# caishiqing/voice-tts

Measured on AMD Instinct MI355X. Metric: audio_seconds_per_second, higher is better.
Workload: dtype bf16

## Files before the change

### include/ixtts_hip.h

```cpp
#ifndef IXTTS_HIP_H
#define IXTTS_HIP_H

#include <stddef.h>
#include <stdint.h>

#ifdef __cplusplus
extern "C" {
#endif

#define IXTTS_OK 0
#define IXTTS_ERR_ARG (-1)
#define IXTTS_ERR_HIP (-2)
#define IXTTS_ERR_STATE (-3)
#define IXTTS_ERR_NOMEM (-4)
#define IXTTS_ERR_NAME (-5)

const char* ixtts_version(void);
const char* ixtts_last_error(void);

int ixtts_aa_snake_f32(const float* x_dev, float* y_dev, const float* up12_dev, const float* down12_dev,
                       const float* log_alpha_dev, const float* log_beta_dev, int B, int C, int T, void* stream);

size_t ixtts_attn_full_workspace_bytes(int B, int H, int T);
int ixtts_attn_full_f32(const float* q_dev, const float* k_dev, const float* v_dev, float* out_dev, int B, int H, int T,
// ... 114 lines not shown
int ixtts_gpt_beam_begin(ixtts_gpt* h, int num_beams, void* stream);
int ixtts_gpt_beam_decode(ixtts_gpt* h, int n_steps, const ixtts_sampler_cfg* sc, void* stream);
int ixtts_gpt_beam_read(ixtts_gpt* h, int max_new, int32_t* ids_host, int cap, int* n_ids, int* done, float* score,
                        float* beam_scores_host, int32_t* last_tokens_host, int32_t* beam_idx_host, void* stream);
int ixtts_gpt_beam_force(ixtts_gpt* h, const int32_t* picks_host, int n, void* stream);

int ixtts_gpt_beam_begin_group(ixtts_gpt* h, int group, int num_beams, uint64_t rng_stream, void* stream);
int ixtts_gpt_beam_park_group(ixtts_gpt* h, int group, void* stream);
int ixtts_gpt_beam_decode_groups(ixtts_gpt* h, int n_groups, int n_steps, const ixtts_sampler_cfg* sc, void* stream);
int ixtts_gpt_beam_read_group(ixtts_gpt* h, int group, int max_new, int32_t* ids_host, int cap, int* n_ids, int* done, float* score,
                              float* beam_scores_host, int32_t* last_tokens_host, int32_t* beam_idx_host, void* stream);
int ixtts_gpt_beam_force_group(ixtts_gpt* h, int group, const int32_t* picks_host, int n, void* stream);

int ixtts_gpt_latent(ixtts_gpt* h, const float* prefix_dev, int n_prefix, const int32_t* codes_dev, int n,
                     float* latent_dev, void* stream);

int ixtts_gpt_bench_gemv(ixtts_gpt* h, int which, int layer, int batch, void* stream);
double ixtts_gpt_step_bytes(const ixtts_gpt* h, int B, int S);

int ixtts_gpt_max_batch(void);

int ixtts_gpt_destroy(ixtts_gpt* h);

#define IXTTS_QWEN_TOPK_MAX 64
#define IXTTS_QWEN_MAX_EOS 8

typedef struct ixtts_qwen_cfg {
  int hidden_size;
  int layers;
  int heads;
// ... 42 lines not shown
```

### voice-tts_amd/_lib.py

```python
import ctypes as C
import os

HERE = os.path.dirname(os.path.abspath(__file__))
LIB_PATH = os.environ.get("IXTTS_LIB") or os.path.join(HERE, "libixtts_hip.so")

MAX_STAGES = 8
MAX_RESK = 4


class BigVGANCfg(C.Structure):
    _fields_ = [
        ("num_mels", C.c_int), ("upsample_initial_channel", C.c_int), ("n_stages", C.c_int),
        ("upsample_rates", C.c_int * MAX_STAGES), ("upsample_kernel_sizes", C.c_int * MAX_STAGES),
        ("n_resblock_kernels", C.c_int), ("resblock_kernel_sizes", C.c_int * MAX_RESK),
        ("resblock_dilations", (C.c_int * 3) * MAX_RESK), ("max_frames", C.c_int), ("fast_sin", C.c_int),
    ]


class GptCfg(C.Structure):
    _fields_ = [
        ("model_dim", C.c_int), ("layers", C.c_int), ("heads", C.c_int), ("n_mel_codes", C.c_int),
        ("n_mel_pos", C.c_int), ("n_text_tokens", C.c_int), ("n_text_pos", C.c_int),
        ("start_mel_token", C.c_int), ("stop_mel_token", C.c_int), ("max_seq", C.c_int),
        ("max_batch", C.c_int), ("weight_dtype", C.c_int),
# ... 75 lines not shown
    "ixtts_gpt_decode": (C.c_int, [_P, C.c_int, C.c_int, C.POINTER(SamplerCfg), _P]),
    "ixtts_gpt_read": (C.c_int, [_P, C.c_int, _P, C.c_int, C.POINTER(C.c_int), C.POINTER(C.c_int), _P]),
    "ixtts_gpt_read_logits": (C.c_int, [_P, C.c_int, _P, _P]),
    "ixtts_gpt_beam_begin": (C.c_int, [_P, C.c_int, _P]),
    "ixtts_gpt_beam_decode": (C.c_int, [_P, C.c_int, C.POINTER(SamplerCfg), _P]),
    "ixtts_gpt_beam_read": (C.c_int, [_P, C.c_int, _P, C.c_int, C.POINTER(C.c_int), C.POINTER(C.c_int), C.POINTER(C.c_float), _P, _P, _P, _P]),
    "ixtts_gpt_beam_force": (C.c_int, [_P, _P, C.c_int, _P]),
    "ixtts_gpt_beam_begin_group": (C.c_int, [_P, C.c_int, C.c_int, C.c_uint64, _P]),
    "ixtts_gpt_beam_park_group": (C.c_int, [_P, C.c_int, _P]),
    "ixtts_gpt_beam_decode_groups": (C.c_int, [_P, C.c_int, C.c_int, C.POINTER(SamplerCfg), _P]),
    "ixtts_gpt_beam_read_group": (C.c_int, [_P, C.c_int, C.c_int, _P, C.c_int, C.POINTER(C.c_int), C.POINTER(C.c_int), C.POINTER(C.c_float), _P, _P, _P, _P]),
    "ixtts_gpt_beam_force_group": (C.c_int, [_P, C.c_int, _P, C.c_int, _P]),
    "ixtts_gpt_read_probs": (C.c_int, [_P, C.c_int, _P, _P]),
    "ixtts_gpt_force_next": (C.c_int, [_P, C.c_int, C.c_int32, _P]),
    "ixtts_gpt_latent": (C.c_int, [_P, _P, C.c_int, _P, C.c_int, _P, _P]),
    "ixtts_gpt_bench_gemv": (C.c_int, [_P, C.c_int, C.c_int, C.c_int, _P]),
    "ixtts_gpt_step_bytes": (C.c_double, [_P, C.c_int, C.c_int]),
    "ixtts_gpt_max_batch": (C.c_int, []),
    "ixtts_gpt_destroy": (C.c_int, [_P]),
    "ixtts_qwen_create": (C.c_int, [C.POINTER(_P), C.POINTER(QwenCfg)]),
    "ixtts_qwen_set_tensor": (C.c_int, [_P, C.c_char_p, _P, C.POINTER(C.c_int64), C.c_int]),
    "ixtts_qwen_finalize": (C.c_int, [_P]),
    "ixtts_qwen_prefill": (C.c_int, [_P, _P, C.c_int, _P]),
    "ixtts_qwen_step": (C.c_int, [_P, C.c_int, C.POINTER(QwenSampling), _P]),
    "ixtts_qwen_read": (C.c_int, [_P, _P, C.c_int, C.POINTER(C.c_int), C.POINTER(C.c_int), _P]),
    "ixtts_qwen_generate": (C.c_int, [_P, C.c_int, C.POINTER(QwenSampling), _P, C.c_int, C.POINTER(C.c_int), C.POINTER(C.c_int), _P]),
    "ixtts_qwen_read_logits": (C.c_int, [_P, _P, _P]),
    "ixtts_qwen_read_kept": (C.c_int, [_P, _P, _P, C.c_int, C.POINTER(C.c_int), _P]),
    "ixtts_qwen_draw": (C.c_int, [_P, C.c_uint64, C.c_int, _P, _P]),
    "ixtts_qwen_step_bytes": (C.c_double, [_P, C.c_int]),
# ... 44 lines not shown
```

### voice-tts_amd/csrc/gpt_engine.h

```cpp
#pragma once
#include <map>
#include <string>
#include <vector>

#include "common.h"

namespace ixtts {

constexpr int MAXB = 16;
constexpr int MAXB_REG = 4;
constexpr int STEPS_PER_GRAPH = 8;
constexpr int BEAM_MAX = 4;
constexpr int MAXG = MAXB / 2;
constexpr int BEAM_LCP_STRIDE = BEAM_MAX * BEAM_MAX + BEAM_MAX;
constexpr int BEAM_FORCED_STRIDE = 2 * BEAM_MAX;

enum TKind { T_VEC = 0, T_MAT_T = 1, T_MAT_N = 2, T_EMB = 3 };

struct TDesc {
  size_t off = 0;
  int kind = T_VEC;
  int64_t d0 = 0, d1 = 0;
  size_t stage_off = 0;
  bool set = false;
// ... 48 lines not shown
  float* probs = nullptr;
  ixtts_sampler_cfg samp_host;
  float* scratch = nullptr;
  size_t scratch_floats = 0;
  hipStream_t cap_stream = nullptr;
  hipGraphExec_t step_exec[ixtts::MAXB + 1][ixtts::NBKT + 1] = {};
  hipGraphExec_t multi_exec[ixtts::MAXB + 1][ixtts::NBKT + 1] = {};
  bool mlp_fused = false;
  void* wprx = nullptr;
  float* mlp_part = nullptr;
  unsigned* mlp_ctr = nullptr;
  float* h2 = nullptr;
  float* hc = nullptr;
  bool wide = false;
  int pf_per = 2;
  bool attn_split = true;
  int attn_bucket = ixtts::NBKT;
  int host_prompt_len[ixtts::MAXB + 2];
  int host_gen_est[ixtts::MAXB + 2];
  int num_beams = 0;
  int beam_groups = 1;
  bool group_live[ixtts::MAXG] = {};
  bool group_begun[ixtts::MAXG] = {};
  unsigned long long* beam_stream = nullptr;
  float *beam_scores = nullptr, *hyp_score = nullptr, *hyp_worst = nullptr;
  int *beam_src = nullptr, *hyp_len = nullptr, *n_hyp = nullptr, *beam_done = nullptr, *beam_forced_flag = nullptr;
  int32_t *hyp_tok = nullptr, *beam_forced = nullptr;
  float* beam_cand_v = nullptr;
  int *beam_cand_i = nullptr, *beam_cand_n = nullptr;
  bool beam_every_row = false;
// ... 22 lines not shown
```

### voice-tts_amd/csrc/gpt_engine.hip

```cpp
#define IXTTS_ENGINE_TU 1
#include <type_traits>

#include "gpt_engine.h"
#include "gpt_kernels.h"
#include "gpt_wide.h"

using namespace ixtts;

#ifdef IXTTS_TRACE
static int g_trace_seq = 0;
#define IXTTS_TRACE_ARG , g_trace_seq++
#else
#define IXTTS_TRACE_ARG
#endif
template <typename WT, typename KVT, int K, int ROWS, int UNITS, int B, int INP, int EPI, int WPB = 4, bool XLDS = false>
static int launch_gemv(const GemvArgs& a, hipStream_t st) {
  auto kern = gemv_reg_kernel<WT, K, ROWS, UNITS, B, INP, EPI, KVT, WPB, XLDS>;
  const int n_units = (a.N + ROWS - 1) / ROWS;
  const int grid = ceil_div(n_units, WPB * UNITS);
  hipLaunchKernelGGL(kern, dim3(grid), dim3(64 * WPB), 0, st, a.wt, a.xin, a.bias, a.out, a.N, a.slot0, a.out_stride, a.smax, a.kcache, a.vcache,
                     a.cur_len, a.heads, a.nsplit, a.ln_w, a.ln_b, a.aux, a.xout IXTTS_PF_ARGS(a) IXTTS_TRACE_ARG);
  return IXTTS_OK;
}

// ... 472 lines not shown
  {
    int ones[MAXG];
    for (int g = 0; g < MAXG; ++g) ones[g] = 1;
    hipMemcpy(h->beam_done, ones, sizeof(ones), hipMemcpyHostToDevice);
    hipMemset(h->beam_forced_flag, 0, MAXG * 4);
    hipMemset(h->beam_stream, 0, MAXG * 8);
    hipMemset(h->n_hyp, 0, MAXG * 4);
    hipMemset(h->beam_lcp, 0, (size_t)MAXG * BEAM_LCP_STRIDE * 4);
    hipMemset(h->beam_src, 0, MAXB * 4);
  }
  if (hipStreamCreateWithFlags(&h->cap_stream, hipStreamNonBlocking) != hipSuccess) return fail("stream");
  if (const char* e = getenv("IXTTS_ATTN")) h->attn_split = strcmp(e, "legacy") != 0;
  h->wide = c->max_batch > MAXB_REG;
  if (const char* e = getenv("IXTTS_WIDE")) h->wide = h->wide || (strcmp(e, "1") == 0 && c->weight_dtype != IXTTS_DTYPE_F32);
  if (const char* e = getenv("IXTTS_BEAM_REORDER")) h->beam_every_row = strcmp(e, "full") == 0;
  if (const char* e = getenv("IXTTS_PF_KIB")) h->pf_per = atoi(e);
  if (h->wide) h->attn_split = false;
  memset(h->host_prompt_len, 0, sizeof(h->host_prompt_len));
  memset(h->host_gen_est, 0, sizeof(h->host_gen_est));
  *out = h;
  return IXTTS_OK;
}

extern "C" int ixtts_gpt_set_tensor(ixtts_gpt* h, const char* name, const float* data, const int64_t* shape, int ndim) {
  IX_ARG(h && name && data && shape, "gpt_set_tensor: null argument");
  auto it = h->tens.find(name);
  if (it == h->tens.end()) {
    set_error("gpt_set_tensor: unknown tensor '%s'", name);
    return IXTTS_ERR_NAME;
  }
// ... 564 lines not shown
  IX_ARG(n + 2 <= h->cfg.n_mel_pos, "gpt_latent: %d codes exceed the mel position table", n);
  IX_ARG(n_prefix + n + 2 < h->smax, "gpt_latent: sequence of %d rows exceeds max_seq %d", n_prefix + n + 2, h->smax);
  if (n == 0) return IXTTS_OK;
  hipStream_t st = (hipStream_t)stream;
  const int D = h->D;
  const int slot = h->slots - 1;
  const int rows = n_prefix + n;
  IX_HIP(hipMemcpyAsync(h->rx, prefix, (size_t)n_prefix * D * 4, hipMemcpyDeviceToDevice, st));
  IX_TRY(embed_mel_rows(h, h->rx + (size_t)n_prefix * D, codes, n, st));
  IX_TRY(forward_rows(h, slot, rows, 0, 0, st));
  IX_TRY(final_norm_rows(h, h->rx + (size_t)n_prefix * D, latent, n, st));
  IX_HIP(hipGetLastError());
  return IXTTS_OK;
}

extern "C" int ixtts_gpt_bench_gemv(ixtts_gpt* h, int which, int layer, int batch, void* stream) {
  NEED_READY(h, "gpt_bench_gemv");
  IX_ARG(layer >= 0 && layer < h->L && batch >= 1 && batch <= h->cfg.max_batch, "gpt_bench_gemv: bad argument");
  return do_gemv_which(h, which, layer, batch, (hipStream_t)stream);
}

extern "C" int ixtts_gpt_max_batch(void) { return MAXB; }

extern "C" double ixtts_gpt_step_bytes(const ixtts_gpt* h, int B, int S) {
  if (!h) return 0.0;
  const double D = h->D, FF = h->FF, V = h->V, L = h->L, es = (double)h->esize;
  double mat = L * (3 * D * D + D * D + 2 * D * FF) + V * D;
  double vec = L * (2 * D + 3 * D + D + 2 * D + FF + D) + 4 * D + V;
  double kv_read = (double)B * 2 * L * S * D * es;
  double kv_write = (double)B * 2 * L * D * es;
// ... 50 lines not shown
```

### voice-tts_amd/csrc/gpt_rows.hip

```cpp
#include "gpt_engine.h"
#include "gpt_kernels.h"

namespace ixtts {

typedef float f32x16 __attribute__((ext_vector_type(16)));
typedef __bf16 bf16x8 __attribute__((ext_vector_type(8)));
typedef _Float16 f16x8 __attribute__((ext_vector_type(8)));

template <typename ET>
struct RowsEl;
template <>
struct RowsEl<bf16> {
  typedef bf16x8 vec8;
  __device__ static __forceinline__ f32x16 mfma(const vec8& a, const vec8& b, const f32x16& c) { return __builtin_amdgcn_mfma_f32_32x32x16_bf16(a, b, c, 0, 0, 0); }
};
template <>
struct RowsEl<f16> {
  typedef f16x8 vec8;
  __device__ static __forceinline__ f32x16 mfma(const vec8& a, const vec8& b, const f32x16& c) { return __builtin_amdgcn_mfma_f32_32x32x16_f16(a, b, c, 0, 0, 0); }
};

__device__ __forceinline__ unsigned int pack_bf16x2(float a, float b) {
  const unsigned short lo = __builtin_bit_cast(unsigned short, (__bf16)a);
  const unsigned short hi = __builtin_bit_cast(unsigned short, (__bf16)b);
// ... 223 lines not shown

struct GemmArgs16 {
  const unsigned short* A;
  const unsigned short* wt;
  const float* bias;
  void* out;
  void* kcache;
  void* vcache;
  int T, N, K, pos0, smax, D;
};

__device__ __forceinline__ void glds16(const void* gsrc, void* lds_wave_base) {
  __builtin_amdgcn_global_load_lds((const __attribute__((address_space(1))) void*)gsrc, (__attribute__((address_space(3))) void*)lds_wave_base, 16, 0, 0);
}

constexpr int G16_NBUF = 2;
constexpr int G16_TILE = 128 * 64 * 2;
constexpr int G16_SMEM = G16_NBUF * 2 * G16_TILE;

template <int EPI, typename KVT>
__global__ __launch_bounds__(256) void gemm_rows_bf16_kernel(GemmArgs16 g) {
  using EL = RowsEl<KVT>;
  typedef typename EL::vec8 vec8;
  constexpr int BM = 128, BN = 128, BK = 64, TILE = G16_TILE, NBUF = G16_NBUF;
  extern __shared__ __attribute__((aligned(1024))) unsigned char smem_raw[];
  unsigned char (*smem)[2][TILE] = reinterpret_cast<unsigned char (*)[2][TILE]>(smem_raw);
  const int tid = threadIdx.x, lane = tid & 63, wave = tid >> 6;
  const int wm = wave >> 1, wn = wave & 1;
  const int l31 = lane & 31, lh = lane >> 5;
  const int m0 = blockIdx.y * BM, n0 = blockIdx.x * BN;

  f32x16 acc[2][2];
#pragma unroll
  for (int mi = 0; mi < 2; ++mi)
#pragma unroll
    for (int j = 0; j < 2; ++j)
#pragma unroll
      for (int r = 0; r < 16; ++r) acc[mi][j][r] = 0.f;

  const unsigned short* asrc[4];
  const unsigned short* wsrc[4];
#pragma unroll
  for (int i = 0; i < 4; ++i) {
    const int row = (wave * 4 + i) * 8 + (lane >> 3);
    const int gran = (lane & 7) ^ ((row >> 1) & 7);
    asrc[i] = g.A + (size_t)min(m0 + row, g.T - 1) * g.K + gran * 8;
    wsrc[i] = g.wt + (size_t)min(n0 + row, g.N - 1) * g.K + gran * 8;
  }
  auto issue = [&](int kt, int buf) {
#pragma unroll
    for (int i = 0; i < 4; ++i) {
      glds16(asrc[i] + kt * BK, &smem[buf][0][(wave * 4 + i) * 1024]);
      glds16(wsrc[i] + kt * BK, &smem[buf][1][(wave * 4 + i) * 1024]);
    }
  };
  const int nkt = g.K / BK;
#pragma unroll
  for (int p = 0; p < NBUF - 1; ++p) issue(min(p, nkt - 1), p);
  for (int kt = 0; kt < nkt; ++kt) {
    issue(min(kt + NBUF - 1, nkt - 1), (kt + NBUF - 1) % NBUF);
    static_assert(NBUF == 2, "the immediate below is 8 * (NBUF - 1)");
    asm volatile("s_waitcnt vmcnt(8)" ::: "memory");
    __builtin_amdgcn_s_barrier();
    const unsigned char* At = smem[kt % NBUF][0];
    const unsigned char* Wt = smem[kt % NBUF][1];
#pragma unroll
    for (int kk = 0; kk < BK / 16; ++kk) {
      vec8 a[2], b[2];
#pragma unroll
      for (int mi = 0; mi < 2; ++mi) {
        const int row = wm * 64 + mi * 32 + l31;
        a[mi] = *reinterpret_cast<const vec8*>(At + row * 128 + (((kk * 2 + lh) ^ ((row >> 1) & 7)) << 4));
      }
#pragma unroll
      for (int j = 0; j < 2; ++j) {
        const int row = wn * 64 + j * 32 + l31;
        b[j] = *reinterpret_cast<const vec8*>(Wt + row * 128 + (((kk * 2 + lh) ^ ((row >> 1) & 7)) << 4));
      }
#pragma unroll
      for (int mi = 0; mi < 2; ++mi)
#pragma unroll
        for (int j = 0; j < 2; ++j) acc[mi][j] = EL::mfma(a[mi], b[j], acc[mi][j]);
    }
    __builtin_amdgcn_s_barrier();
  }
  float bias[2];
  int ncol[2];
#pragma unroll
  for (int j = 0; j < 2; ++j) {
    ncol[j] = n0 + wn * 64 + j * 32 + l31;
    bias[j] = g.bias[min(ncol[j], g.N - 1)];
  }
  if constexpr (EPI == RE_RESID) {
    float* xo = reinterpret_cast<float*>(g.out);
    float old[2][2][16];
#pragma unroll
    for (int mi = 0; mi < 2; ++mi)
#pragma unroll
      for (int j = 0; j < 2; ++j)
#pragma unroll
        for (int r = 0; r < 16; ++r) {
          const int m = min(m0 + wm * 64 + mi * 32 + (r & 3) + 8 * (r >> 2) + 4 * lh, g.T - 1);
          old[mi][j][r] = xo[(size_t)m * g.N + min(ncol[j], g.N - 1)];
        }
#pragma unroll
    for (int mi = 0; mi < 2; ++mi)
#pragma unroll
      for (int j = 0; j < 2; ++j)
#pragma unroll
        for (int r = 0; r < 16; ++r) {
          const int m = m0 + wm * 64 + mi * 32 + (r & 3) + 8 * (r >> 2) + 4 * lh;
          if (m < g.T && ncol[j] < g.N) xo[(size_t)m * g.N + ncol[j]] = old[mi][j][r] + (acc[mi][j][r] + bias[j]);
        }
  } else {
#pragma unroll
    for (int mi = 0; mi < 2; ++mi)
#pragma unroll
      for (int j = 0; j < 2; ++j) {
        const int n = ncol[j];
#pragma unroll
        for (int r = 0; r < 16; ++r) {
          const int m = m0 + wm * 64 + mi * 32 + (r & 3) + 8 * (r >> 2) + 4 * lh;
          if (m >= g.T || n >= g.N) continue;
          const float v = acc[mi][j][r] + bias[j];
          if constexpr (EPI == RE_GELU) {
            const float u2 = 1.5957691216057308f * (v + 0.044715f * v * v * v);
            store_kv(reinterpret_cast<KVT*>(g.out) + (size_t)m * g.N + n, v / (1.0f + __expf(-u2)));
          } else {
            if (n < g.D) {
              reinterpret_cast<float*>(g.out)[(size_t)m * g.D + n] = v;
            } else {
              const int which = n / g.D;
              const int c = n - which * g.D;
              const int hh = c / HD, d = c % HD;
              KVT* cache = reinterpret_cast<KVT*>(which == 1 ? g.kcache : g.vcache);
              store_kv(cache + ((size_t)hh * g.smax + g.pos0 + m) * HD + d, v);
            }
// ... 53 lines not shown
    const uint4 r = reinterpret_cast<const uint4*>(p)[i];
    v[8 * i] = lo_f16(r.x); v[8 * i + 1] = hi_f16(r.x); v[8 * i + 2] = lo_f16(r.y); v[8 * i + 3] = hi_f16(r.y);
    v[8 * i + 4] = lo_f16(r.z); v[8 * i + 5] = hi_f16(r.z); v[8 * i + 6] = lo_f16(r.w); v[8 * i + 7] = hi_f16(r.w);
  }
}
template <>
__device__ __forceinline__ void load_row16<bf16>(const bf16* p, float (&v)[16]) {
#pragma unroll
  for (int i = 0; i < 2; ++i) {
    const uint4 r = reinterpret_cast<const uint4*>(p)[i];
    v[8 * i] = lo_bf16(r.x); v[8 * i + 1] = hi_bf16(r.x); v[8 * i + 2] = lo_bf16(r.y); v[8 * i + 3] = hi_bf16(r.y);
    v[8 * i + 4] = lo_bf16(r.z); v[8 * i + 5] = hi_bf16(r.z); v[8 * i + 6] = lo_bf16(r.w); v[8 * i + 7] = hi_bf16(r.w);
  }
}

template <typename KVT, typename OT>
__global__ __launch_bounds__(256) void attn_rows_flash_kernel(AttnRowsArgs a) {
  __shared__ __attribute__((aligned(16))) float Ks[FR_KT * FR_KP];
  __shared__ __attribute__((aligned(16))) float Vs[FR_KT * HD];
  const int hh = blockIdx.x;
  const int lane = threadIdx.x & 63, wave = threadIdx.x >> 6;
  const int l31 = lane & 31, lh = lane >> 5;
  const int qw0 = blockIdx.y * 128 + wave * 32;
  const KVT* kb = reinterpret_cast<const KVT*>(a.kcache) + (size_t)hh * a.smax * HD;
  const KVT* vb = reinterpret_cast<const KVT*>(a.vcache) + (size_t)hh * a.smax * HD;
  const int last_key = a.pos0 + a.T - 1;

  float qr[HD / 2];
  {
    const int qi = min(qw0 + l31, a.T - 1);
    const float* qp = a.q + (size_t)qi * a.D + hh * HD + 4 * lh;
    const float qs = 0.125f * 1.4426950408889634f;
#pragma unroll
    for (int m = 0; m < HD / 8; ++m) {
      const float4 t = *reinterpret_cast<const float4*>(qp + 8 * m);
      qr[4 * m] = t.x * qs; qr[4 * m + 1] = t.y * qs; qr[4 * m + 2] = t.z * qs; qr[4 * m + 3] = t.w * qs;
    }
  }
  f32x16 ot[2];
#pragma unroll
  for (int j = 0; j < 2; ++j)
#pragma unroll
    for (int r = 0; r < 16; ++r) ot[j][r] = 0.f;
  float m_run = -INFINITY, l_run = 0.f;
  const int lim = a.pos0 + qw0 + l31;
  const int wave_lim = a.pos0 + min(qw0 + 31, a.T - 1);
  const int wg_lim = a.pos0 + min((int)blockIdx.y * 128 + 127, a.T - 1);
  const int t_first = (a.valid_from / FR_KT) * FR_KT;

  for (int t0 = t_first; t0 <= wg_lim; t0 += FR_KT) {
    __syncthreads();
    {
      const int key = threadIdx.x >> 2, c16 = (threadIdx.x & 3) * 16;
      const int t = min(max(t0 + key, a.valid_from), last_key);
      float kv[16], vv[16];
      load_row16<KVT>(kb + (size_t)t * HD + c16, kv);
      load_row16<KVT>(vb + (size_t)t * HD + c16, vv);
#pragma unroll
      for (int i = 0; i < 4; ++i) {
        *reinterpret_cast<float4*>(Ks + key * FR_KP + c16 + 4 * i) = make_float4(kv[4 * i], kv[4 * i + 1], kv[4 * i + 2], kv[4 * i + 3]);
        *reinterpret_cast<float4*>(Vs + key * HD + c16 + 4 * i) = make_float4(vv[4 * i], vv[4 * i + 1], vv[4 * i + 2], vv[4 * i + 3]);
      }
    }
    __syncthreads();
    if (t0 > wave_lim) continue;

    f32x16 st[2];
#pragma unroll
    for (int j = 0; j < 2; ++j)
#pragma unroll
      for (int r = 0; r < 16; ++r) st[j][r] = 0.f;
    const float* kp0 = Ks + l31 * FR_KP + 4 * lh;
    const float* kp1 = kp0 + 32 * FR_KP;
    float4 ka[2][2];
    ka[0][0] = *reinterpret_cast<const float4*>(kp0);
    ka[0][1] = *reinterpret_cast<const float4*>(kp1);
#pragma unroll
    for (int m = 0; m < HD / 8; ++m) {
      if (m + 1 < HD / 8) {
// ... 62 lines not shown
      ot[0] = __builtin_amdgcn_mfma_f32_32x32x2f32(va[s2 & 1][0], pv, ot[0], 0, 0, 0);
      ot[1] = __builtin_amdgcn_mfma_f32_32x32x2f32(va[s2 & 1][1], pv, ot[1], 0, 0, 0);
    }
  }
  const int qi = qw0 + l31;
  if (qi < a.T) {
    const float inv = l_run > 0.f ? 1.0f / l_run : 0.f;
    OT* op = reinterpret_cast<OT*>(a.out) + (size_t)qi * a.D + hh * HD;
#pragma unroll
    for (int j = 0; j < 2; ++j)
#pragma unroll
      for (int r = 0; r < 16; ++r) store_kv(op + j * 32 + (r & 3) + 8 * (r >> 2) + 4 * lh, ot[j][r] * inv);
  }
}

template <typename KVT, typename OT>
static void launch_attn_rows(ixtts_gpt* h, const AttnRowsArgs& a, hipStream_t st) {
  static const bool legacy = getenv("IXTTS_ROWS_ATTN") && !strcmp(getenv("IXTTS_ROWS_ATTN"), "legacy");
  if (legacy) hipLaunchKernelGGL((attn_rows_kernel<KVT, OT>), dim3(h->H, a.T), dim3(256), 0, st, a);
  else hipLaunchKernelGGL((attn_rows_flash_kernel<KVT, OT>), dim3(h->H, ceil_div(a.T, 128)), dim3(256), 0, st, a);
}

template <typename WT, typename KVT, int EPI>
static void launch_gemm(const GemmArgs& g, hipStream_t st) {
  if (g.T >= 512) {
    hipLaunchKernelGGL((gemm_rows_kernel<WT, EPI, KVT, 128>), dim3(ceil_div(g.N, GBN), ceil_div(g.T, 128)), dim3(256), 0, st, g);
  } else {
    hipLaunchKernelGGL((gemm_rows_kernel<WT, EPI, KVT, 64>), dim3(ceil_div(g.N, GBN), ceil_div(g.T, 64)), dim3(256), 0, st, g);
  }
}

template <typename WT, typename KVT, int D>
static int forward_rows_t(ixtts_gpt* h, int slot, int T, int pos0, int valid_from, hipStream_t st) {
  const size_t lstride = (size_t)h->slots * D * h->smax * sizeof(KVT);
  const size_t sstride = (size_t)D * h->smax * sizeof(KVT);
// ... 9 lines not shown
    AttnRowsArgs a;
    a.q = h->rq; a.kcache = kc; a.vcache = vc; a.out = h->ratt; a.T = T; a.D = D; a.smax = h->smax; a.pos0 = pos0; a.valid_from = valid_from;
    launch_attn_rows<KVT, float>(h, a, st);
    g.A = h->ratt; g.wt = A_PTR(o.wo); g.bias = A_F32(o.bo); g.out = h->rx; g.N = D; g.K = D;
    launch_gemm<WT, KVT, RE_RESID>(g, st);
    hipLaunchKernelGGL(ln_rows_kernel<D>, dim3(ceil_div(T, 4)), dim3(256), 0, st, h->rx, h->rxn, T);
    g.A = h->rxn; g.wt = A_PTR(o.wfc); g.bias = A_F32(o.bfc); g.out = h->rff; g.N = 4 * D; g.K = D;
    launch_gemm<WT, KVT, RE_GELU>(g, st);
    g.A = h->rff; g.wt = A_PTR(o.wpr); g.bias = A_F32(o.bpr); g.out = h->rx; g.N = D; g.K = 4 * D;
    launch_gemm<WT, KVT, RE_RESID>(g, st);
  }
  IX_HIP(hipGetLastError());
  return IXTTS_OK;
}

template <typename KVT, int D>
static int forward_rows_16(ixtts_gpt* h, int slot, int T, int pos0, int valid_from, hipStream_t st) {
  const size_t lstride = (size_t)h->slots * D * h->smax * sizeof(KVT);
  const size_t sstride = (size_t)D * h->smax * sizeof(KVT);
  KVT* xn16 = reinterpret_cast<KVT*>(h->rxn);
  KVT* att16 = reinterpret_cast<KVT*>(h->ratt);
  KVT* ff16 = reinterpret_cast<KVT*>(h->rff);
  const dim3 blk(256);
  auto grid = [&](int N) { return dim3(ceil_div(N, 128), ceil_div(T, 128)); };
  static bool attr_done = false;
  if (!attr_done) {
    IX_HIP(hipFuncSetAttribute((const void*)gemm_rows_bf16_kernel<RE_QKV, KVT>, hipFuncAttributeMaxDynamicSharedMemorySize, G16_SMEM));
    IX_HIP(hipFuncSetAttribute((const void*)gemm_rows_bf16_kernel<RE_RESID, KVT>, hipFuncAttributeMaxDynamicSharedMemorySize, G16_SMEM));
    IX_HIP(hipFuncSetAttribute((const void*)gemm_rows_bf16_kernel<RE_GELU, KVT>, hipFuncAttributeMaxDynamicSharedMemorySize, G16_SMEM));
    attr_done = true;
  }
  for (int l = 0; l < h->L; ++l) {
    const LayerOff& o = h->lo[l];
    uint8_t* kc = (uint8_t*)h->kc + l * lstride + slot * sstride;
    uint8_t* vc = (uint8_t*)h->vc + l * lstride + slot * sstride;
    hipLaunchKernelGGL((ln_rows_kernel<D, KVT>), dim3(ceil_div(T, 4)), blk, 0, st, h->rx, xn16, T);
    GemmArgs16 g;
    g.A = reinterpret_cast<const unsigned short*>(xn16); g.wt = reinterpret_cast<const unsigned short*>(A_PTR(o.wqkv)); g.bias = A_F32(o.bqkv);
    g.out = h->rq; g.kcache = kc; g.vcache = vc; g.T = T; g.N = 3 * D; g.K = D; g.pos0 = pos0; g.smax = h->smax; g.D = D;
    hipLaunchKernelGGL((gemm_rows_bf16_kernel<RE_QKV, KVT>), grid(g.N), blk, G16_SMEM, st, g);
    AttnRowsArgs a;
    a.q = h->rq; a.kcache = kc; a.vcache = vc; a.out = att16; a.T = T; a.D = D; a.smax = h->smax; a.pos0 = pos0; a.valid_from = valid_from;
    launch_attn_rows<KVT, KVT>(h, a, st);
    g.A = reinterpret_cast<const unsigned short*>(att16); g.wt = reinterpret_cast<const unsigned short*>(A_PTR(o.wo)); g.bias = A_F32(o.bo);
    g.out = h->rx; g.N = D; g.K = D;
    hipLaunchKernelGGL((gemm_rows_bf16_kernel<RE_RESID, KVT>), grid(g.N), blk, G16_SMEM, st, g);
    hipLaunchKernelGGL((ln_rows_kernel<D, KVT>), dim3(ceil_div(T, 4)), blk, 0, st, h->rx, xn16, T);
    g.A = reinterpret_cast<const unsigned short*>(xn16); g.wt = reinterpret_cast<const unsigned short*>(A_PTR(o.wfc)); g.bias = A_F32(o.bfc);
    g.out = ff16; g.N = 4 * D; g.K = D;
    hipLaunchKernelGGL((gemm_rows_bf16_kernel<RE_GELU, KVT>), grid(g.N), blk, G16_SMEM, st, g);
    g.A = reinterpret_cast<const unsigned short*>(ff16); g.wt = reinterpret_cast<const unsigned short*>(A_PTR(o.wpr)); g.bias = A_F32(o.bpr);
    g.out = h->rx; g.N = D; g.K = 4 * D;
    hipLaunchKernelGGL((gemm_rows_bf16_kernel<RE_RESID, KVT>), grid(g.N), blk, G16_SMEM, st, g);
  }
  IX_HIP(hipGetLastError());
  return IXTTS_OK;
}

int forward_rows(ixtts_gpt* h, int slot, int T, int pos0, int valid_from, hipStream_t st) {
  if (T <= 0) return IXTTS_OK;
  if (h->cfg.weight_dtype == IXTTS_DTYPE_F32) {
    return h->D == 1280 ? forward_rows_t<float, float, 1280>(h, slot, T, pos0, valid_from, st)
                        : forward_rows_t<float, float, 128>(h, slot, T, pos0, valid_from, st);
  }
  if (h->cfg.weight_dtype == IXTTS_DTYPE_F16)
    return h->D == 1280 ? forward_rows_16<f16, 1280>(h, slot, T, pos0, valid_from, st) : forward_rows_16<f16, 128>(h, slot, T, pos0, valid_from, st);
  return h->D == 1280 ? forward_rows_16<bf16, 1280>(h, slot, T, pos0, valid_from, st) : forward_rows_16<bf16, 128>(h, slot, T, pos0, valid_from, st);
}
// ... 31 lines not shown
```

### voice-tts_amd/gpt_engine.py

```python
import ctypes as C

import numpy as np
import torch

from . import _lib
from .weights import GPT_CFG

GPT_DTYPES = {"f32": 0, "bf16": 1, "f16": 2}


def _dtype_code(dtype):
    if dtype not in GPT_DTYPES:
        raise ValueError(f"GPT weight dtype {dtype!r}: expected one of " + ", ".join(GPT_DTYPES))
    return GPT_DTYPES[dtype]


def resolve_gpt_dtype(use_fp16, gpt_dtype=None, env=None):
    import os

    if gpt_dtype is None:
        gpt_dtype = (os.environ if env is None else env).get("IXTTS_GPT_DTYPE") or None
        if gpt_dtype is not None:
            gpt_dtype = gpt_dtype.strip().lower()
    if gpt_dtype is None:
# ... 136 lines not shown
        src = np.zeros(self._nb, np.int32)
        with torch.cuda.device(self.device):
            rc = _lib.lib().ixtts_gpt_beam_read_group(self._h, int(group), int(max_new), ids.ctypes.data, ids.size, C.byref(n), C.byref(done), C.byref(score),
                                                      bs.ctypes.data, lt.ctypes.data, src.ctypes.data, self._stream())
        _lib.check(rc, "ixtts_gpt_beam_read_group")
        return ids[: n.value].copy(), bool(done.value), float(score.value), bs, lt, src

    def latent(self, prefix, codes):
        p = prefix.to(self.device, torch.float32).contiguous()
        c = codes.to(self.device, torch.int32).contiguous()
        out = torch.empty(c.numel(), self.D, device=self.device, dtype=torch.float32)
        with torch.cuda.device(self.device):
            rc = _lib.lib().ixtts_gpt_latent(self._h, p.data_ptr(), p.shape[0], c.data_ptr(), c.numel(), out.data_ptr(), self._stream())
        _lib.check(rc, "ixtts_gpt_latent")
        self._keep2 = (p, c)
        return out

    def step_bytes(self, B, S):
        return _lib.lib().ixtts_gpt_step_bytes(self._h, B, S)

    def bench_gemv(self, which, layer, batch=1):
        with torch.cuda.device(self.device):
            _lib.check(_lib.lib().ixtts_gpt_bench_gemv(self._h, which, layer, batch, self._stream()), "ixtts_gpt_bench_gemv")

    def store_mel_emb(self, mel_emb):
        self.cached_mel_emb = mel_emb

    def generate(self, inputs, bos_token_id=None, pad_token_id=None, eos_token_id=None, attention_mask=None,
                 max_length=None, logits_processor=None, num_return_sequences=1, do_sample=True, top_p=1.0, top_k=0,
                 temperature=1.0, num_beams=1, repetition_penalty=1.0, length_penalty=0.0, sync_every=64,
# ... 86 lines not shown
```

Baseline: 41.31.

## Pick GEMM row tile shape by grid size and prefetch KV in flash attention

Parameterizes the prefill rows GEMM over tile shape and buffer count, adding 128x64 and 64x64 tiles with deeper pipelines and an M-fast grid. A heuristic picks the smaller tiles when the legacy 128x128 grid would launch too few workgroups to fill the GPU. The flash attention rows kernel now prefetches the next K/V tile into registers while computing the current one, and schedules row blocks in reverse order. A debug peek API and an IXTTS_ROWS=legacy fallback are also added. Smaller tiles reuse less data per load and add register pressure.

```diff
diff --git a/include/ixtts_hip.h b/include/ixtts_hip.h
--- a/include/ixtts_hip.h
+++ b/include/ixtts_hip.h
@@ -152,6 +152,8 @@
 
 int ixtts_gpt_latent(ixtts_gpt* h, const float* prefix_dev, int n_prefix, const int32_t* codes_dev, int n,
                      float* latent_dev, void* stream);
+
+int ixtts_gpt_peek(ixtts_gpt* h, int what, int layer, int slot, void* out_host, size_t bytes, void* stream);
 
 int ixtts_gpt_bench_gemv(ixtts_gpt* h, int which, int layer, int batch, void* stream);
 double ixtts_gpt_step_bytes(const ixtts_gpt* h, int B, int S);
diff --git a/voice-tts_amd/_lib.py b/voice-tts_amd/_lib.py
--- a/voice-tts_amd/_lib.py
+++ b/voice-tts_amd/_lib.py
@@ -113,6 +113,7 @@
     "ixtts_gpt_read_probs": (C.c_int, [_P, C.c_int, _P, _P]),
     "ixtts_gpt_force_next": (C.c_int, [_P, C.c_int, C.c_int32, _P]),
     "ixtts_gpt_latent": (C.c_int, [_P, _P, C.c_int, _P, C.c_int, _P, _P]),
+    "ixtts_gpt_peek": (C.c_int, [_P, C.c_int, C.c_int, C.c_int, _P, C.c_size_t, _P]),
     "ixtts_gpt_bench_gemv": (C.c_int, [_P, C.c_int, C.c_int, C.c_int, _P]),
     "ixtts_gpt_step_bytes": (C.c_double, [_P, C.c_int, C.c_int]),
     "ixtts_gpt_max_batch": (C.c_int, []),
diff --git a/voice-tts_amd/csrc/gpt_engine.h b/voice-tts_amd/csrc/gpt_engine.h
--- a/voice-tts_amd/csrc/gpt_engine.h
+++ b/voice-tts_amd/csrc/gpt_engine.h
@@ -86,6 +86,7 @@
   float* hc = nullptr;
   bool wide = false;
   int pf_per = 2;
+  bool rows_legacy = false;
   bool attn_split = true;
   int attn_bucket = ixtts::NBKT;
   int host_prompt_len[ixtts::MAXB + 2];
diff --git a/voice-tts_amd/csrc/gpt_engine.hip b/voice-tts_amd/csrc/gpt_engine.hip
--- a/voice-tts_amd/csrc/gpt_engine.hip
+++ b/voice-tts_amd/csrc/gpt_engine.hip
@@ -510,6 +510,7 @@
   h->wide = c->max_batch > MAXB_REG;
   if (const char* e = getenv("IXTTS_WIDE")) h->wide = h->wide || (strcmp(e, "1") == 0 && c->weight_dtype != IXTTS_DTYPE_F32);
   if (const char* e = getenv("IXTTS_BEAM_REORDER")) h->beam_every_row = strcmp(e, "full") == 0;
+  if (const char* e = getenv("IXTTS_ROWS")) h->rows_legacy = strcmp(e, "legacy") == 0;
   if (const char* e = getenv("IXTTS_PF_KIB")) h->pf_per = atoi(e);
   if (h->wide) h->attn_split = false;
   memset(h->host_prompt_len, 0, sizeof(h->host_prompt_len));
@@ -1104,6 +1105,25 @@
   return IXTTS_OK;
 }
 
+extern "C" int ixtts_gpt_peek(ixtts_gpt* h, int what, int layer, int slot, void* out_host, size_t bytes, void* stream) {
+  NEED_READY(h, "gpt_peek");
+  IX_ARG(out_host && what >= 0 && what <= 2, "gpt_peek: bad argument");
+  const uint8_t* src;
+  size_t cap;
+  if (what == 0) {
+    src = reinterpret_cast<const uint8_t*>(h->rx);
+    cap = (size_t)h->smax * h->D * 4;
+  } else {
+    IX_ARG(layer >= 0 && layer < h->L && slot >= 0 && slot < h->slots, "gpt_peek: layer %d / slot %d out of range", layer, slot);
+    cap = (size_t)h->D * h->smax * h->esize;
+    src = reinterpret_cast<const uint8_t*>(what == 1 ? h->kc : h->vc) + ((size_t)layer * h->slots + slot) * cap;
+  }
+  IX_ARG(bytes <= cap, "gpt_peek: %zu bytes asked of a region of %zu", bytes, cap);
+  IX_HIP(hipStreamSynchronize((hipStream_t)stream));
+  IX_HIP(hipMemcpy(out_host, src, bytes, hipMemcpyDeviceToHost));
+  return IXTTS_OK;
+}
+
 extern "C" int ixtts_gpt_bench_gemv(ixtts_gpt* h, int which, int layer, int batch, void* stream) {
   NEED_READY(h, "gpt_bench_gemv");
   IX_ARG(layer >= 0 && layer < h->L && batch >= 1 && batch <= h->cfg.max_batch, "gpt_bench_gemv: bad argument");
diff --git a/voice-tts_amd/csrc/gpt_rows.hip b/voice-tts_amd/csrc/gpt_rows.hip
--- a/voice-tts_amd/csrc/gpt_rows.hip
+++ b/voice-tts_amd/csrc/gpt_rows.hip
@@ -261,44 +261,61 @@
   __builtin_amdgcn_global_load_lds((const __attribute__((address_space(1))) void*)gsrc, (__attribute__((address_space(3))) void*)lds_wave_base, 16, 0, 0);
 }
 
-constexpr int G16_NBUF = 2;
-constexpr int G16_TILE = 128 * 64 * 2;
-constexpr int G16_SMEM = G16_NBUF * 2 * G16_TILE;
-
-template <int EPI, typename KVT>
+template <int BM_, int BN_, int NBUF_, bool MFAST_>
+struct RowsTile {
+  static constexpr int BM = BM_, BN = BN_, NBUF = NBUF_;
+  static constexpr bool MFAST = MFAST_;
+  static constexpr int TILE_A = BM * 128, TILE_W = BN * 128;
+  static constexpr int STAGE = TILE_A + TILE_W;
+  static constexpr int SMEM = NBUF * STAGE;
+  static constexpr int PA = BM / 32, PW = BN / 32;
+  static constexpr int MI = BM / 64, NJ = BN / 64;
+  static_assert(BM % 64 == 0 && BN % 64 == 0 && NBUF >= 2 && (PA + PW) * (NBUF - 1) < 64, "tile");
+};
+typedef RowsTile<128, 128, 2, false> RT_Legacy;
+typedef RowsTile<128, 64, 3, true> RT_HalfN;
+typedef RowsTile<64, 64, 4, true> RT_Small;
+
+template <int EPI, typename KVT, typename TL = RT_Legacy>
 __global__ __launch_bounds__(256) void gemm_rows_bf16_kernel(GemmArgs16 g) {
   using EL = RowsEl<KVT>;
   typedef typename EL::vec8 vec8;
-  constexpr int BM = 128, BN = 128, BK = 64, TILE = G16_TILE, NBUF = G16_NBUF;
+  constexpr int BM = TL::BM, BN = TL::BN, BK = 64, NBUF = TL::NBUF, MI = TL::MI, NJ = TL::NJ, PA = TL::PA, PW = TL::PW;
   extern __shared__ __attribute__((aligned(1024))) unsigned char smem_raw[];
-  unsigned char (*smem)[2][TILE] = reinterpret_cast<unsigned char (*)[2][TILE]>(smem_raw);
   const int tid = threadIdx.x, lane = tid & 63, wave = tid >> 6;
   const int wm = wave >> 1, wn = wave & 1;
   const int l31 = lane & 31, lh = lane >> 5;
-  const int m0 = blockIdx.y * BM, n0 = blockIdx.x * BN;
-
-  f32x16 acc[2][2];
-#pragma unroll
-  for (int mi = 0; mi < 2; ++mi)
-#pragma unroll
-    for (int j = 0; j < 2; ++j)
+  const int m0 = (TL::MFAST ? blockIdx.x : blockIdx.y) * BM, n0 = (TL::MFAST ? blockIdx.y : blockIdx.x) * BN;
+
+  f32x16 acc[MI][NJ];
+#pragma unroll
+  for (int mi = 0; mi < MI; ++mi)
+#pragma unroll
+    for (int j = 0; j < NJ; ++j)
 #pragma unroll
       for (int r = 0; r < 16; ++r) acc[mi][j][r] = 0.f;
 
-  const unsigned short* asrc[4];
-  const unsigned short* wsrc[4];
-#pragma unroll
-  for (int i = 0; i < 4; ++i) {
-    const int row = (wave * 4 + i) * 8 + (lane >> 3);
+  const unsigned short* asrc[PA];
+  const unsigned short* wsrc[PW];
+#pragma unroll
+  for (int i = 0; i < PA; ++i) {
+    const int row = (wave * PA + i) * 8 + (lane >> 3);
     const int gran = (lane & 7) ^ ((row >> 1) & 7);
     asrc[i] = g.A + (size_t)min(m0 + row, g.T - 1) * g.K + gran * 8;
+  }
+#pragma unroll
+  for (int i = 0; i < PW; ++i) {
+    const int row = (wave * PW + i) * 8 + (lane >> 3);
+    const int gran = (lane & 7) ^ ((row >> 1) & 7);
     wsrc[i] = g.wt + (size_t)min(n0 + row, g.N - 1) * g.K + gran * 8;
   }
   auto issue = [&](int kt, int buf) {
-#pragma unroll
-    for (int i = 0; i < 4; ++i) {
-      glds16(asrc[i] + kt * BK, &smem[buf][0][(wave * 4 + i) * 1024]);
-      glds16(wsrc[i] + kt * BK, &smem[buf][1][(wave * 4 + i) * 1024]);
+    unsigned char* sa = smem_raw + buf * TL::STAGE;
+    unsigned char* sw = sa + TL::TILE_A;
+#pragma unroll
+    for (int i = 0; i < (PA > PW ? PA : PW); ++i) {
+      if (i < PA) glds16(asrc[i] + kt * BK, sa + (wave * PA + i) * 1024);
+      if (i < PW) glds16(wsrc[i] + kt * BK, sw + (wave * PW + i) * 1024);
     }
   };
   const int nkt = g.K / BK;
@@ -306,68 +323,68 @@
   for (int p = 0; p < NBUF - 1; ++p) issue(min(p, nkt - 1), p);
   for (int kt = 0; kt < nkt; ++kt) {
     issue(min(kt + NBUF - 1, nkt - 1), (kt + NBUF - 1) % NBUF);
-    static_assert(NBUF == 2, "the immediate below is 8 * (NBUF - 1)");
-    asm volatile("s_waitcnt vmcnt(8)" ::: "memory");
+    asm volatile("s_waitcnt vmcnt(%0)" ::"n"((PA + PW) * (NBUF - 1)) : "memory");
     __builtin_amdgcn_s_barrier();
-    const unsigned char* At = smem[kt % NBUF][0];
-    const unsigned char* Wt = smem[kt % NBUF][1];
+    const unsigned char* At = smem_raw + (kt % NBUF) * TL::STAGE;
+    const unsigned char* Wt = At + TL::TILE_A;
 #pragma unroll
     for (int kk = 0; kk < BK / 16; ++kk) {
-      vec8 a[2], b[2];
-#pragma unroll
-      for (int mi = 0; mi < 2; ++mi) {
-        const int row = wm * 64 + mi * 32 + l31;
+      vec8 a[MI], b[NJ];
+#pragma unroll
+      for (int mi = 0; mi < MI; ++mi) {
+        const int row = wm * (BM / 2) + mi * 32 + l31;
         a[mi] = *reinterpret_cast<const vec8*>(At + row * 128 + (((kk * 2 + lh) ^ ((row >> 1) & 7)) << 4));
       }
 #pragma unroll
-      for (int j = 0; j < 2; ++j) {
-        const int row = wn * 64 + j * 32 + l31;
+      for (int j = 0; j < NJ; ++j) {
+        const int row = wn * (BN / 2) + j * 32 + l31;
         b[j] = *reinterpret_cast<const vec8*>(Wt + row * 128 + (((kk * 2 + lh) ^ ((row >> 1) & 7)) << 4));
       }
 #pragma unroll
-      for (int mi = 0; mi < 2; ++mi)
-#pragma unroll
-        for (int j = 0; j < 2; ++j) acc[mi][j] = EL::mfma(a[mi], b[j], acc[mi][j]);
+      for (int mi = 0; mi < MI; ++mi)
+#pragma unroll
+        for (int j = 0; j < NJ; ++j) acc[mi][j] = EL::mfma(a[mi], b[j], acc[mi][j]);
     }
     __builtin_amdgcn_s_barrier();
   }
-  float bias[2];
-  int ncol[2];
-#pragma unroll
-  for (int j = 0; j < 2; ++j) {
-    ncol[j] = n0 + wn * 64 + j * 32 + l31;
+  float bias[NJ];
+  int ncol[NJ];
+#pragma unroll
+  for (int j = 0; j < NJ; ++j) {
+    ncol[j] = n0 + wn * (BN / 2) + j * 32 + l31;
     bias[j] = g.bias[min(ncol[j], g.N - 1)];
   }
+  const int mw0 = m0 + wm * (BM / 2);
   if constexpr (EPI == RE_RESID) {
     float* xo = reinterpret_cast<float*>(g.out);
-    float old[2][2][16];
-#pragma unroll
-    for (int mi = 0; mi < 2; ++mi)
-#pragma unroll
-      for (int j = 0; j < 2; ++j)
+    float old[MI][NJ][16];
+#pragma unroll
+    for (int mi = 0; mi < MI; ++mi)
+#pragma unroll
+      for (int j = 0; j < NJ; ++j)
 #pragma unroll
         for (int r = 0; r < 16; ++r) {
-          const int m = min(m0 + wm * 64 + mi * 32 + (r & 3) + 8 * (r >> 2) + 4 * lh, g.T - 1);
+          const int m = min(mw0 + mi * 32 + (r & 3) + 8 * (r >> 2) + 4 * lh, g.T - 1);
           old[mi][j][r] = xo[(size_t)m * g.N + min(ncol[j], g.N - 1)];
         }
 #pragma unroll
-    for (int mi = 0; mi < 2; ++mi)
-#pragma unroll
-      for (int j = 0; j < 2; ++j)
+    for (int mi = 0; mi < MI; ++mi)
+#pragma unroll
+      for (int j = 0; j < NJ; ++j)
 #pragma unroll
         for (int r = 0; r < 16; ++r) {
-          const int m = m0 + wm * 64 + mi * 32 + (r & 3) + 8 * (r >> 2) + 4 * lh;
+          const int m = mw0 + mi * 32 + (r & 3) + 8 * (r >> 2) + 4 * lh;
           if (m < g.T && ncol[j] < g.N) xo[(size_t)m * g.N + ncol[j]] = old[mi][j][r] + (acc[mi][j][r] + bias[j]);
         }
   } else {
 #pragma unroll
-    for (int mi = 0; mi < 2; ++mi)
-#pragma unroll
-      for (int j = 0; j < 2; ++j) {
+    for (int mi = 0; mi < MI; ++mi)
+#pragma unroll
+      for (int j = 0; j < NJ; ++j) {
         const int n = ncol[j];
 #pragma unroll
         for (int r = 0; r < 16; ++r) {
-          const int m = m0 + wm * 64 + mi * 32 + (r & 3) + 8 * (r >> 2) + 4 * lh;
+          const int m = mw0 + mi * 32 + (r & 3) + 8 * (r >> 2) + 4 * lh;
           if (m >= g.T || n >= g.N) continue;
           const float v = acc[mi][j][r] + bias[j];
           if constexpr (EPI == RE_GELU) {
@@ -451,14 +468,38 @@
   }
 }
 
-template <typename KVT, typename OT>
+template <typename KVT>
+struct Raw16 {
+  uint4 r[2];
+  __device__ __forceinline__ void load(const KVT* p) {
+    r[0] = reinterpret_cast<const uint4*>(p)[0];
+    r[1] = reinterpret_cast<const uint4*>(p)[1];
+  }
+  __device__ __forceinline__ void widen(float (&v)[16]) const {
+#pragma unroll
+    for (int i = 0; i < 2; ++i) {
+      const unsigned w[4] = {r[i].x, r[i].y, r[i].z, r[i].w};
+#pragma unroll
+      for (int c = 0; c < 4; ++c) {
+        if constexpr (__is_same(KVT, f16)) {
+          v[8 * i + 2 * c] = lo_f16(w[c]); v[8 * i + 2 * c + 1] = hi_f16(w[c]);
+        } else {
+          v[8 * i + 2 * c] = lo_bf16(w[c]); v[8 * i + 2 * c + 1] = hi_bf16(w[c]);
+        }
+      }
+    }
+  }
+};
+
+template <typename KVT, typename OT, bool FILL = false>
 __global__ __launch_bounds__(256) void attn_rows_flash_kernel(AttnRowsArgs a) {
   __shared__ __attribute__((aligned(16))) float Ks[FR_KT * FR_KP];
   __shared__ __attribute__((aligned(16))) float Vs[FR_KT * HD];
   const int hh = blockIdx.x;
+  const int rb = FILL ? (int)(gridDim.y - 1 - blockIdx.y) : (int)blockIdx.y;
   const int lane = threadIdx.x & 63, wave = threadIdx.x >> 6;
   const int l31 = lane & 31, lh = lane >> 5;
-  const int qw0 = blockIdx.y * 128 + wave * 32;
+  const int qw0 = rb * 128 + wave * 32;
   const KVT* kb = reinterpret_cast<const KVT*>(a.kcache) + (size_t)hh * a.smax * HD;
   const KVT* vb = reinterpret_cast<const KVT*>(a.vcache) + (size_t)hh * a.smax * HD;
   const int last_key = a.pos0 + a.T - 1;
@@ -482,24 +523,38 @@
   float m_run = -INFINITY, l_run = 0.f;
   const int lim = a.pos0 + qw0 + l31;
   const int wave_lim = a.pos0 + min(qw0 + 31, a.T - 1);
-  const int wg_lim = a.pos0 + min((int)blockIdx.y * 128 + 127, a.T - 1);
+  const int wg_lim = a.pos0 + min(rb * 128 + 127, a.T - 1);
   const int t_first = (a.valid_from / FR_KT) * FR_KT;
+
+  const int skey = threadIdx.x >> 2, sc16 = (threadIdx.x & 3) * 16;
+  Raw16<KVT> kraw, vraw;
+  auto fetch = [&](int t0) {
+    const int t = min(max(t0 + skey, a.valid_from), last_key);
+    kraw.load(kb + (size_t)t * HD + sc16);
+    vraw.load(vb + (size_t)t * HD + sc16);
+  };
+  if constexpr (FILL) fetch(t_first);
 
   for (int t0 = t_first; t0 <= wg_lim; t0 += FR_KT) {
     __syncthreads();
     {
-      const int key = threadIdx.x >> 2, c16 = (threadIdx.x & 3) * 16;
-      const int t = min(max(t0 + key, a.valid_from), last_key);
       float kv[16], vv[16];
-      load_row16<KVT>(kb + (size_t)t * HD + c16, kv);
-      load_row16<KVT>(vb + (size_t)t * HD + c16, vv);
+      if constexpr (FILL) {
+        kraw.widen(kv);
+        vraw.widen(vv);
+      } else {
+        const int t = min(max(t0 + skey, a.valid_from), last_key);
+        load_row16<KVT>(kb + (size_t)t * HD + sc16, kv);
+        load_row16<KVT>(vb + (size_t)t * HD + sc16, vv);
+      }
 #pragma unroll
       for (int i = 0; i < 4; ++i) {
-        *reinterpret_cast<float4*>(Ks + key * FR_KP + c16 + 4 * i) = make_float4(kv[4 * i], kv[4 * i + 1], kv[4 * i + 2], kv[4 * i + 3]);
-        *reinterpret_cast<float4*>(Vs + key * HD + c16 + 4 * i) = make_float4(vv[4 * i], vv[4 * i + 1], vv[4 * i + 2], vv[4 * i + 3]);
+        *reinterpret_cast<float4*>(Ks + skey * FR_KP + sc16 + 4 * i) = make_float4(kv[4 * i], kv[4 * i + 1], kv[4 * i + 2], kv[4 * i + 3]);
+        *reinterpret_cast<float4*>(Vs + skey * HD + sc16 + 4 * i) = make_float4(vv[4 * i], vv[4 * i + 1], vv[4 * i + 2], vv[4 * i + 3]);
       }
     }
     __syncthreads();
+    if constexpr (FILL) fetch(t0 + FR_KT);
     if (t0 > wave_lim) continue;
 
     f32x16 st[2];
@@ -592,11 +647,11 @@
   }
 }
 
-template <typename KVT, typename OT>
+template <typename KVT, typename OT, bool FILL = false>
 static void launch_attn_rows(ixtts_gpt* h, const AttnRowsArgs& a, hipStream_t st) {
   static const bool legacy = getenv("IXTTS_ROWS_ATTN") && !strcmp(getenv("IXTTS_ROWS_ATTN"), "legacy");
   if (legacy) hipLaunchKernelGGL((attn_rows_kernel<KVT, OT>), dim3(h->H, a.T), dim3(256), 0, st, a);
-  else hipLaunchKernelGGL((attn_rows_flash_kernel<KVT, OT>), dim3(h->H, ceil_div(a.T, 128)), dim3(256), 0, st, a);
+  else hipLaunchKernelGGL((attn_rows_flash_kernel<KVT, OT, FILL>), dim3(h->H, ceil_div(a.T, 128)), dim3(256), 0, st, a);
 }
 
 template <typename WT, typename KVT, int EPI>
@@ -636,6 +691,41 @@
   return IXTTS_OK;
 }
 
+enum { RT_LEGACY = 0, RT_HALFN = 1, RT_SMALL = 2 };
+static int rows_tile(int T, int N) {
+  const int mt = ceil_div(T, 128);
+  if (mt * ceil_div(N, 128) >= 256) return RT_LEGACY;
+  if (mt * ceil_div(N, 64) >= 200) return RT_HALFN;
+  return RT_SMALL;
+}
+
+template <int EPI, typename KVT, typename TL>
+static void launch_gemm16_tile(const GemmArgs16& g, hipStream_t st) {
+  const int mt = ceil_div(g.T, TL::BM), nt = ceil_div(g.N, TL::BN);
+  hipLaunchKernelGGL((gemm_rows_bf16_kernel<EPI, KVT, TL>), TL::MFAST ? dim3(mt, nt) : dim3(nt, mt), dim3(256), TL::SMEM, st, g);
+}
+
+template <int EPI, typename KVT>
+static void launch_gemm16(const ixtts_gpt* h, const GemmArgs16& g, hipStream_t st) {
+  const int tile = h->rows_legacy ? RT_LEGACY : rows_tile(g.T, g.N);
+  if (tile == RT_LEGACY) launch_gemm16_tile<EPI, KVT, RT_Legacy>(g, st);
+  else if (tile == RT_HALFN) launch_gemm16_tile<EPI, KVT, RT_HalfN>(g, st);
+  else launch_gemm16_tile<EPI, KVT, RT_Small>(g, st);
+}
+
+template <int EPI, typename KVT, typename TL>
+static int gemm16_attr() {
+  IX_HIP(hipFuncSetAttribute((const void*)gemm_rows_bf16_kernel<EPI, KVT, TL>, hipFuncAttributeMaxDynamicSharedMemorySize, TL::SMEM));
+  return IXTTS_OK;
+}
+template <typename KVT, typename TL>
+static int gemm16_attrs() {
+  IX_TRY((gemm16_attr<RE_QKV, KVT, TL>()));
+  IX_TRY((gemm16_attr<RE_RESID, KVT, TL>()));
+  IX_TRY((gemm16_attr<RE_GELU, KVT, TL>()));
+  return IXTTS_OK;
+}
+
 template <typename KVT, int D>
 static int forward_rows_16(ixtts_gpt* h, int slot, int T, int pos0, int valid_from, hipStream_t st) {
   const size_t lstride = (size_t)h->slots * D * h->smax * sizeof(KVT);
@@ -644,12 +734,11 @@
   KVT* att16 = reinterpret_cast<KVT*>(h->ratt);
   KVT* ff16 = reinterpret_cast<KVT*>(h->rff);
   const dim3 blk(256);
-  auto grid = [&](int N) { return dim3(ceil_div(N, 128), ceil_div(T, 128)); };
   static bool attr_done = false;
   if (!attr_done) {
-    IX_HIP(hipFuncSetAttribute((const void*)gemm_rows_bf16_kernel<RE_QKV, KVT>, hipFuncAttributeMaxDynamicSharedMemorySize, G16_SMEM));
-    IX_HIP(hipFuncSetAttribute((const void*)gemm_rows_bf16_kernel<RE_RESID, KVT>, hipFuncAttributeMaxDynamicSharedMemorySize, G16_SMEM));
-    IX_HIP(hipFuncSetAttribute((const void*)gemm_rows_bf16_kernel<RE_GELU, KVT>, hipFuncAttributeMaxDynamicSharedMemorySize, G16_SMEM));
+    IX_TRY((gemm16_attrs<KVT, RT_Legacy>()));
+    IX_TRY((gemm16_attrs<KVT, RT_HalfN>()));
+    IX_TRY((gemm16_attrs<KVT, RT_Small>()));
     attr_done = true;
   }
   for (int l = 0; l < h->L; ++l) {
@@ -660,20 +749,21 @@
     GemmArgs16 g;
     g.A = reinterpret_cast<const unsigned short*>(xn16); g.wt = reinterpret_cast<const unsigned short*>(A_PTR(o.wqkv)); g.bias = A_F32(o.bqkv);
     g.out = h->rq; g.kcache = kc; g.vcache = vc; g.T = T; g.N = 3 * D; g.K = D; g.pos0 = pos0; g.smax = h->smax; g.D = D;
-    hipLaunchKernelGGL((gemm_rows_bf16_kernel<RE_QKV, KVT>), grid(g.N), blk, G16_SMEM, st, g);
+    launch_gemm16<RE_QKV, KVT>(h, g, st);
     AttnRowsArgs a;
     a.q = h->rq; a.kcache = kc; a.vcache = vc; a.out = att16; a.T = T; a.D = D; a.smax = h->smax; a.pos0 = pos0; a.valid_from = valid_from;
-    launch_attn_rows<KVT, KVT>(h, a, st);
+    if (h->rows_legacy) launch_attn_rows<KVT, KVT>(h, a, st);
+    else launch_attn_rows<KVT, KVT, true>(h, a, st);
     g.A = reinterpret_cast<const unsigned short*>(att16); g.wt = reinterpret_cast<const unsigned short*>(A_PTR(o.wo)); g.bias = A_F32(o.bo);
     g.out = h->rx; g.N = D; g.K = D;
-    hipLaunchKernelGGL((gemm_rows_bf16_kernel<RE_RESID, KVT>), grid(g.N), blk, G16_SMEM, st, g);
+    launch_gemm16<RE_RESID, KVT>(h, g, st);
     hipLaunchKernelGGL((ln_rows_kernel<D, KVT>), dim3(ceil_div(T, 4)), blk, 0, st, h->rx, xn16, T);
     g.A = reinterpret_cast<const unsigned short*>(xn16); g.wt = reinterpret_cast<const unsigned short*>(A_PTR(o.wfc)); g.bias = A_F32(o.bfc);
     g.out = ff16; g.N = 4 * D; g.K = D;
-    hipLaunchKernelGGL((gemm_rows_bf16_kernel<RE_GELU, KVT>), grid(g.N), blk, G16_SMEM, st, g);
+    launch_gemm16<RE_GELU, KVT>(h, g, st);
     g.A = reinterpret_cast<const unsigned short*>(ff16); g.wt = reinterpret_cast<const unsigned short*>(A_PTR(o.wpr)); g.bias = A_F32(o.bpr);
     g.out = h->rx; g.N = D; g.K = 4 * D;
-    hipLaunchKernelGGL((gemm_rows_bf16_kernel<RE_RESID, KVT>), grid(g.N), blk, G16_SMEM, st, g);
+    launch_gemm16<RE_RESID, KVT>(h, g, st);
   }
   IX_HIP(hipGetLastError());
   return IXTTS_OK;
diff --git a/voice-tts_amd/gpt_engine.py b/voice-tts_amd/gpt_engine.py
--- a/voice-tts_amd/gpt_engine.py
+++ b/voice-tts_amd/gpt_engine.py
@@ -174,6 +174,13 @@
             rc = _lib.lib().ixtts_gpt_latent(self._h, p.data_ptr(), p.shape[0], c.data_ptr(), c.numel(), out.data_ptr(), self._stream())
         _lib.check(rc, "ixtts_gpt_latent")
         self._keep2 = (p, c)
+        return out
+
+    def peek(self, what, layer=0, slot=0, nbytes=0):
+        out = np.zeros(nbytes, dtype=np.uint8)
+        with torch.cuda.device(self.device):
+            rc = _lib.lib().ixtts_gpt_peek(self._h, {"rows": 0, "k": 1, "v": 2}[what], layer, slot, out.ctypes.data, nbytes, self._stream())
+        _lib.check(rc, "ixtts_gpt_peek")
         return out
 
     def step_bytes(self, B, S):
```

Result: no change. 41.50 (median of 6 runs) (+0.4%).
